# nerfstudio-project/nerfstudio

Hardware: AMD Instinct MI355X
Metric: training rays/sec (4096 rays x 48 samples per GPU) (higher is better)
Workload: dtype f32

## Files before the change

### nerfstudio_amd/csrc/density_mlp.hip

```cpp
#include "common.h"
#include "launch.h"
#include "mfma_chain.h"
#include "proposal_chain.h"

namespace nsamd {

constexpr int kMlpBlock = 256;
constexpr int kMaxBlocks = 768;
constexpr int kDensityActMax = 2048;

__host__ __device__ constexpr int density_partial_stride(int in_dim, int hidden) {
  return (hidden * in_dim + 2 * hidden + 1 + 3) & ~3;
}

template <int IN, int H>
__global__ __launch_bounds__(kMlpBlock) void density_mlp_fwd_kernel(const float* __restrict__ enc,
                                                                    const float* __restrict__ selector, int64_t M,
                                                                    nsamd_density_mlp mlp,
                                                                    float* __restrict__ density,
                                                                    float* __restrict__ pre_out) {
  const float* __restrict__ W0 = mlp.W0;
  const float* __restrict__ b0 = mlp.b0;
  const float* __restrict__ W1 = mlp.W1;
  for (int64_t p = (int64_t)blockIdx.x * kMlpBlock + threadIdx.x; p < M; p += (int64_t)gridDim.x * kMlpBlock) {
    float x[IN];
#pragma unroll
    for (int k = 0; k < IN; ++k) x[k] = enc[(int64_t)k * M + p];
    float out = mlp.b1[0];
    constexpr int JU = (H <= 16) ? H : 4;
#pragma unroll JU
    for (int j = 0; j < H; ++j) {
      float a = b0[j];
#pragma unroll
      for (int k = 0; k < IN; ++k) a = fmaf(W0[j * IN + k], x[k], a);
      out = fmaf(W1[j], fmaxf(a, 0.0f), out);
    }
    const float sel = selector ? selector[p] : 1.0f;
    if (pre_out) pre_out[p] = out;
    density[p] = mlp.average_init_density * expf(out) * sel;
  }
}

template <int LEVELS, int H>
__device__ __forceinline__ void density_point(float x, float y, float z, int64_t p, int64_t M, int transform, const nsamd_aabb& box,
                                              const float2* __restrict__ table, const nsamd_grid& grid,
                                              const nsamd_density_mlp& mlp, float* __restrict__ enc_out,
                                              float* __restrict__ selector_out, float* __restrict__ density,
                                              float* __restrict__ pre_out) {
  constexpr int IN = 2 * LEVELS;
  const float sel = normalise_position(transform, box, x, y, z);
  const uint32_t mask = (1u << grid.log2_table_size) - 1u;
  float2 v[LEVELS][8];
  float w[LEVELS][3];
#pragma unroll
  for (int l = 0; l < LEVELS; ++l) {
    const Cell c = locate_cell(x, y, z, grid.scalings[l]);
    w[l][0] = c.w[0]; w[l][1] = c.w[1]; w[l][2] = c.w[2];
    const float2* __restrict__ tl = table + ((size_t)l << grid.log2_table_size);
#pragma unroll
    for (int k = 0; k < 8; ++k) v[l][k] = tl[corner_index(c, k, mask)];
  }
  float feat[IN];
#pragma unroll
  for (int l = 0; l < LEVELS; ++l) {
#pragma unroll
    for (int f = 0; f < 2; ++f)
      feat[2 * l + f] = trilinear_blend([&](int k) { return f == 0 ? v[l][k].x : v[l][k].y; }, w[l][0], w[l][1], w[l][2]);
  }
  if (enc_out != nullptr) {
#pragma unroll
    for (int k = 0; k < IN; ++k) enc_out[(int64_t)k * M + p] = feat[k];
  }
  if (selector_out != nullptr) selector_out[p] = sel;
  const float* __restrict__ W0 = mlp.W0;
  const float* __restrict__ b0 = mlp.b0;
  const float* __restrict__ W1 = mlp.W1;
  float out = mlp.b1[0];
#pragma unroll
  for (int j = 0; j < H; ++j) {
    float a = b0[j];
#pragma unroll
    for (int k = 0; k < IN; ++k) a = fmaf(W0[j * IN + k], feat[k], a);
    out = fmaf(W1[j], fmaxf(a, 0.0f), out);
  }
  if (pre_out != nullptr) pre_out[p] = out;
  density[p] = mlp.average_init_density * expf(out) * sel;
}

template <int LEVELS, int H>
__global__ __launch_bounds__(kMlpBlock) void density_field_fwd_kernel(nsamd_points P, int64_t M, int transform,
                                                                      nsamd_aabb box, const float2* __restrict__ table,
                                                                      nsamd_grid grid, nsamd_density_mlp mlp,
                                                                      float* __restrict__ enc_out,
                                                                      float* __restrict__ selector_out,
                                                                      float* __restrict__ density,
                                                                      float* __restrict__ pre_out) {
  const int64_t p = (int64_t)blockIdx.x * kMlpBlock + threadIdx.x;
  if (p >= M) return;
  float x, y, z;
  load_position(P, p, x, y, z);
  density_point<LEVELS, H>(x, y, z, p, M, transform, box, table, grid, mlp, enc_out, selector_out, density, pre_out);
}

template <int IN, int H>
__device__ __forceinline__ void density_mlp_bwd_body(
    const float* __restrict__ enc, const float* __restrict__ selector, const float* __restrict__ pre,
    const float* __restrict__ ddensity, int64_t M, const nsamd_density_mlp& mlp, float* __restrict__ denc,
    float* __restrict__ dW0, float* __restrict__ db0, float* __restrict__ dW1, float* __restrict__ db1,
    float* __restrict__ partials, const uint32_t* __restrict__ gate, const uint8_t* __restrict__ ray_mask, int spr,
    int nblocks) {
  if (gate != nullptr && __hip_atomic_load(gate, __ATOMIC_RELAXED, __HIP_MEMORY_SCOPE_AGENT) == 0u) return;
  constexpr int LD = kMlpBlock + 1;
  extern __shared__ __attribute__((aligned(16))) float lds[];
  float* gh_T = lds;
  float* x_T = lds + H * LD;
  float* hg_T = x_T + IN * LD;
  float* gp = hg_T + H * LD;
  constexpr int INP = (IN + 3) & ~3;
  float* w0s = lds + (((2 * H + IN + 1) * LD + 3) & ~3);
  float* b0s = w0s + H * INP;
  float* w1s = b0s + H;
  const int64_t chunks = (M + kMlpBlock - 1) / kMlpBlock;
  const int64_t per_wg = (chunks + nblocks - 1) / nblocks;
  const int64_t c_lo = (int64_t)blockIdx.x * per_wg;
  const int64_t c_hi = c_lo + per_wg < chunks ? c_lo + per_wg : chunks;
  constexpr int kActMax = kDensityActMax;
  uint8_t* act = reinterpret_cast<uint8_t*>(w0s + H * INP + 2 * H);
  const bool use_act = ray_mask != nullptr && per_wg <= kActMax;
  if (use_act) {
    for (int64_t k = threadIdx.x; k < per_wg; k += kMlpBlock) act[k] = 0;
    __syncthreads();
    bool any = false;
    if (c_lo < c_hi) {
      const int64_t p_first = c_lo * kMlpBlock, p_last = (c_hi * kMlpBlock < M ? c_hi * kMlpBlock : M) - 1;
      const int64_t r_first = p_first / spr, r_last = p_last / spr;
      for (int64_t r = r_first + threadIdx.x; r <= r_last; r += kMlpBlock) {
        if (ray_mask[r] != 0) {
          any = true;
          const int64_t q0 = r * spr > p_first ? r * spr : p_first, q1 = (r + 1) * spr - 1 < p_last ? (r + 1) * spr - 1 : p_last;
          for (int64_t c = q0 / kMlpBlock; c <= q1 / kMlpBlock; ++c) act[c - c_lo] = 1;
        }
      }
    }
    if (!__syncthreads_or(any)) {
      if (partials != nullptr) {
        float* row = partials + (size_t)blockIdx.x * density_partial_stride(IN, H);
        for (int e = threadIdx.x; e < H * IN + 2 * H + 1; e += kMlpBlock) row[e] = 0.0f;
      }
      return;
    }
  }
  for (int e = threadIdx.x; e < H * INP; e += kMlpBlock) {
    const int j = e / INP, k = e - j * INP;
    w0s[e] = k < IN ? mlp.W0[j * IN + k] : 0.0f;
  }
  bool w_finite = true;
  for (int e = threadIdx.x; e < H * INP; e += kMlpBlock) w_finite = w_finite && fabsf(w0s[e]) <= 3.4028234663852886e38f;
  for (int e = threadIdx.x; e < H; e += kMlpBlock) {
    b0s[e] = mlp.b0[e];
    w1s[e] = mlp.W1[e];
    w_finite = w_finite && fabsf(b0s[e]) <= 3.4028234663852886e38f && fabsf(w1s[e]) <= 3.4028234663852886e38f;
  }
  const bool may_skip = __syncthreads_and(w_finite) != 0;

  constexpr int NT = H / 16;
  static_assert(H % 16 == 0 && IN <= 16, "dW0 tiling");
  v4f accM[NT];
#pragma unroll
  for (int n = 0; n < NT; ++n) accM[n] = v4f{0.f, 0.f, 0.f, 0.f};
  const int lane = threadIdx.x & 63, wv = threadIdx.x >> 6, jj = lane & 15, gg = lane >> 4;
  float accV = 0.0f;

  float x_next[IN];
  float gd_next = 0.0f, sel_next = 1.0f, pre_next = 0.0f;
  bool act_next = true;
  auto chunk_active = [&](int64_t c) {
    if (ray_mask == nullptr) return true;
    if (use_act) return act[c - c_lo] != 0;
    const int64_t p0 = c * kMlpBlock, p1 = (p0 + kMlpBlock < M ? p0 + kMlpBlock : M) - 1;
    bool any = false;
    for (int64_t r = p0 / spr; r <= p1 / spr; ++r) any = any || ray_mask[r] != 0;
    return any;
  };
  auto fetch = [&](int64_t c) {
    const int64_t p = c * kMlpBlock + threadIdx.x;
    act_next = c < c_hi && chunk_active(c);
    const bool live = act_next && p < M;
#pragma unroll
    for (int k = 0; k < IN; ++k) x_next[k] = live ? enc[(int64_t)k * M + p] : 0.0f;
    gd_next = live ? ddensity[p] : 0.0f;
    sel_next = (live && selector) ? selector[p] : 1.0f;
    pre_next = live ? pre[p] : 0.0f;
  };
  fetch(c_lo);
  for (int64_t c = c_lo; c < c_hi; ++c) {
    if (!act_next) {
      fetch(c + 1);
      continue;
    }
    const int64_t p = c * kMlpBlock + threadIdx.x;
    const bool live = p < M;
    float x[IN];
#pragma unroll
    for (int k = 0; k < IN; ++k) x[k] = x_next[k];
    const float g_pre =
        live ? gd_next * sel_next * mlp.average_init_density * expf(fminf(fmaxf(pre_next, -15.0f), 15.0f)) : 0.0f;
    {
      bool carries = g_pre != 0.0f || !may_skip;
#pragma unroll
      for (int k = 0; k < IN; ++k) carries = carries || !(fabsf(x[k]) <= 3.4028234663852886e38f);
      if (!__syncthreads_or(carries)) {
        if (live) {
#pragma unroll
          for (int k = 0; k < IN; ++k) denc[(int64_t)k * M + p] = 0.0f;
        }
        fetch(c + 1);
        continue;
      }
    }
    float dx[IN];
#pragma unroll
    for (int k = 0; k < IN; ++k) dx[k] = 0.0f;
#pragma unroll 4
    for (int j = 0; j < H; ++j) {
      float wj[INP];
#pragma unroll
      for (int k4 = 0; k4 < INP; k4 += 4) {
        const float4 w4 = *reinterpret_cast<const float4*>(w0s + j * INP + k4);
        wj[k4] = w4.x; wj[k4 + 1] = w4.y; wj[k4 + 2] = w4.z; wj[k4 + 3] = w4.w;
      }
      float a = b0s[j];
#pragma unroll
      for (int k = 0; k < IN; ++k) a = fmaf(wj[k], x[k], a);
      const float gh = (a > 0.0f) ? g_pre * w1s[j] : 0.0f;
      gh_T[j * LD + threadIdx.x] = gh;
      hg_T[j * LD + threadIdx.x] = fmaxf(a, 0.0f) * g_pre;
#pragma unroll
      for (int k = 0; k < IN; ++k) dx[k] = fmaf(gh, wj[k], dx[k]);
    }
#pragma unroll
    for (int k = 0; k < IN; ++k) {
      x_T[k * LD + threadIdx.x] = x[k];
      if (live) denc[(int64_t)k * M + p] = dx[k];
    }
    gp[threadIdx.x] = g_pre;
    __syncthreads();
    fetch(c + 1);
#pragma unroll 4
    for (int q = 0; q < 16; ++q) {
      const int pt = 64 * wv + 4 * q + gg;
      const float b = jj < IN ? x_T[jj * LD + pt] : 0.0f;
#pragma unroll
      for (int n = 0; n < NT; ++n)
        accM[n] = mfma16(gh_T[(16 * n + jj) * LD + pt], b, accM[n]);
    }
    if (threadIdx.x < 2 * H + 1) {
      const float* a = (threadIdx.x < H)       ? gh_T + threadIdx.x * LD
                       : (threadIdx.x < 2 * H) ? hg_T + (threadIdx.x - H) * LD
                                               : gp;
      float s = 0.0f;
#pragma unroll 8
      for (int q = 0; q < kMlpBlock; ++q) s += a[q];
      accV += s;
    }
    __syncthreads();
  }
  float* red = lds;
  for (int e = threadIdx.x; e < H * 16; e += kMlpBlock) red[e] = 0.0f;
  __syncthreads();
  for (int turn = 0; turn < kMlpBlock / 64; ++turn) {
    if (wv == turn) {
#pragma unroll
      for (int n = 0; n < NT; ++n)
#pragma unroll
        for (int r = 0; r < 4; ++r) red[(16 * n + 4 * gg + r) * 16 + jj] += accM[n][r];
    }
    __syncthreads();
  }
  if (partials != nullptr) {
    float* row = partials + (size_t)blockIdx.x * density_partial_stride(IN, H);
    for (int e = threadIdx.x; e < H * IN; e += kMlpBlock) row[e] = red[(e / IN) * 16 + (e % IN)];
    if (threadIdx.x < 2 * H + 1) row[H * IN + threadIdx.x] = accV;
    return;
  }
  for (int e = threadIdx.x; e < H * IN; e += kMlpBlock) unsafeAtomicAdd(dW0 + e, red[(e / IN) * 16 + (e % IN)]);
  if (threadIdx.x < H) unsafeAtomicAdd(db0 + threadIdx.x, accV);
  else if (threadIdx.x < 2 * H) unsafeAtomicAdd(dW1 + (threadIdx.x - H), accV);
  else if (threadIdx.x == 2 * H) unsafeAtomicAdd(db1, accV);
}

template <int IN, int H>
__global__ __launch_bounds__(kMlpBlock) void density_mlp_bwd_kernel(
    const float* __restrict__ enc, const float* __restrict__ selector, const float* __restrict__ pre,
    const float* __restrict__ ddensity, int64_t M, nsamd_density_mlp mlp, float* __restrict__ denc,
    float* __restrict__ dW0, float* __restrict__ db0, float* __restrict__ dW1, float* __restrict__ db1,
    float* __restrict__ partials, const uint32_t* __restrict__ gate, const uint8_t* __restrict__ ray_mask, int spr) {
  density_mlp_bwd_body<IN, H>(enc, selector, pre, ddensity, M, mlp, denc, dW0, db0, dW1, db1, partials, gate, ray_mask, spr,
                              (int)gridDim.x);
}

struct DensityBwdArgs {
  const float* enc;
  const float* selector;
  const float* pre;
  const float* ddensity;
  int64_t M;
  nsamd_density_mlp mlp;
  float* denc;
  float* dW0;
  float* db0;
  float* dW1;
  float* db1;
  float* partials;
  const uint32_t* gate;
  const uint8_t* ray_mask;
  int spr;
  int nblocks;
};

template <int IN, int H>
__global__ __launch_bounds__(kMlpBlock) void density_mlp_bwd_pair_kernel(DensityBwdArgs a, DensityBwdArgs b) {
  if (blockIdx.y == 0) {
    if ((int)blockIdx.x >= a.nblocks) return;
    density_mlp_bwd_body<IN, H>(a.enc, a.selector, a.pre, a.ddensity, a.M, a.mlp, a.denc, a.dW0, a.db0, a.dW1, a.db1,
                                a.partials, a.gate, a.ray_mask, a.spr, a.nblocks);
  } else {
    if ((int)blockIdx.x >= b.nblocks) return;
    density_mlp_bwd_body<IN, H>(b.enc, b.selector, b.pre, b.ddensity, b.M, b.mlp, b.denc, b.dW0, b.db0, b.dW1, b.db1,
                                b.partials, b.gate, b.ray_mask, b.spr, b.nblocks);
  }
}

constexpr int kDwGroups = 16;
__device__ __forceinline__ void density_dw_reduce_body(const float* __restrict__ partials, int rows, int stride, int n_w0,
                                                       int hidden, float* __restrict__ dW0, float* __restrict__ db0,
                                                       float* __restrict__ dW1, float* __restrict__ db1,
                                                       const uint32_t* __restrict__ gate) {
  if (gate != nullptr && __hip_atomic_load(gate, __ATOMIC_RELAXED, __HIP_MEMORY_SCOPE_AGENT) == 0u) return;
  __shared__ float part[kDwGroups][64];
  const int el = threadIdx.x & 63, grp = threadIdx.x >> 6;
  const int e = blockIdx.x * 64 + el;
  const int total = n_w0 + 2 * hidden + 1;
  float s = 0.f;
  if (e < total) {
    for (int b0i = grp; b0i < rows; b0i += kDwGroups * 16) {
      float v[16];
#pragma unroll
      for (int u = 0; u < 16; ++u) {
        const int b = b0i + u * kDwGroups;
        v[u] = partials[(size_t)(b < rows ? b : rows - 1) * stride + e];
      }
#pragma unroll
      for (int u = 0; u < 16; ++u) s += (b0i + u * kDwGroups < rows) ? v[u] : 0.0f;
    }
  }
  part[grp][el] = s;
  __syncthreads();
  if (grp == 0 && e < total) {
    float t = 0.f;
#pragma unroll
    for (int g2 = 0; g2 < kDwGroups; ++g2) t += part[g2][el];
    float* dst = e < n_w0 ? dW0 + e : (e < n_w0 + hidden ? db0 + (e - n_w0) : (e < n_w0 + 2 * hidden ? dW1 + (e - n_w0 - hidden) : db1));
    *dst += t;
  }
}

__global__ __launch_bounds__(64 * kDwGroups) void density_dw_reduce_kernel(const float* __restrict__ partials, int rows,
                                                                            int stride, int n_w0, int hidden,
                                                                            float* __restrict__ dW0,
                                                                            float* __restrict__ db0,
                                                                            float* __restrict__ dW1,
                                                                            float* __restrict__ db1,
                                                                            const uint32_t* __restrict__ gate) {
  density_dw_reduce_body(partials, rows, stride, n_w0, hidden, dW0, db0, dW1, db1, gate);
}

__global__ __launch_bounds__(64 * kDwGroups) void density_dw_reduce_pair_kernel(DensityBwdArgs a, DensityBwdArgs b, int stride,
                                                                                 int n_w0, int hidden) {
  if (blockIdx.y == 0) density_dw_reduce_body(a.partials, a.nblocks, stride, n_w0, hidden, a.dW0, a.db0, a.dW1, a.db1, a.gate);
  else density_dw_reduce_body(b.partials, b.nblocks, stride, n_w0, hidden, b.dW0, b.db0, b.dW1, b.db1, b.gate);
}

template <int IN, int H>
static int launch_fwd(const float* enc, const float* selector, int64_t M, nsamd_density_mlp mlp, float* density,
                      float* pre, hipStream_t stream) {
  const unsigned blocks = (unsigned)min((int64_t)8192, (M + kMlpBlock - 1) / kMlpBlock);
  density_mlp_fwd_kernel<IN, H><<<blocks, kMlpBlock, 0, stream>>>(enc, selector, M, mlp, density, pre);
  NSAMD_CHECK_LAUNCH();
  return NSAMD_OK;
}

#define NSAMD_DENSITY_DISPATCH(CALL)                                  \
  if (mlp.in_dim == 10 && mlp.hidden == 16) return CALL(10, 16);      \
  if (mlp.in_dim == 16 && mlp.hidden == 16) return CALL(16, 16);      \
  if (mlp.in_dim == 10 && mlp.hidden == 64) return CALL(10, 64);      \
  if (mlp.in_dim == 16 && mlp.hidden == 64) return CALL(16, 64);      \
  return NSAMD_ERR_UNSUPPORTED;

template <int IN, int H>
static int launch_bwd(const DensityBwdCall* c, int n, hipStream_t stream) {
  constexpr int stride = density_partial_stride(IN, H);
  constexpr int total = H * IN + 2 * H + 1;
  const size_t lds = sizeof(float) * ((size_t)(2 * H + IN + 1) * (kMlpBlock + 1) + 8 + (size_t)H * (((IN + 3) & ~3) + 2)) +
                     kDensityActMax;
  DensityBwdArgs k[2];
  for (int i = 0; i < n; ++i) {
    const int blocks = (int)min((int64_t)kMaxBlocks, (c[i].M + kMlpBlock - 1) / kMlpBlock);
    float* partials = (c[i].workspace != nullptr && c[i].workspace_floats >= (int64_t)blocks * stride) ? c[i].workspace : nullptr;
    k[i] = DensityBwdArgs{c[i].enc, c[i].selector, c[i].pre, c[i].ddensity, c[i].M, c[i].mlp, c[i].denc, c[i].dW0, c[i].db0,
                          c[i].dW1, c[i].db1, partials, c[i].gate, c[i].ray_mask, c[i].ray_mask ? c[i].spr : 1, blocks};
  }
  const bool pair = n == 2 && k[0].partials != nullptr && k[1].partials != nullptr && k[0].partials != k[1].partials &&
                    k[0].dW0 != k[1].dW0;
  if (n == 2 && !pair) {
    const int rc = launch_bwd<IN, H>(c, 1, stream);
    return rc ? rc : launch_bwd<IN, H>(c + 1, 1, stream);
  }
  if (lds > 64 * 1024) {
    static LdsOptIn opted_in;
    const int rc = lds_opt_in(opted_in, density_mlp_bwd_pair_kernel<IN, H>, lds, density_mlp_bwd_kernel<IN, H>, lds);
    if (rc) return rc;
  }
  const DensityBwdArgs& a = k[0];
  if (pair) {
    density_mlp_bwd_pair_kernel<IN, H><<<dim3((unsigned)max(a.nblocks, k[1].nblocks), 2u), kMlpBlock, lds, stream>>>(a, k[1]);
    NSAMD_CHECK_LAUNCH();
    density_dw_reduce_pair_kernel<<<dim3((total + 63) / 64, 2u), 64 * kDwGroups, 0, stream>>>(a, k[1], stride, H * IN, H);
    NSAMD_CHECK_LAUNCH();
    return NSAMD_OK;
  }
  density_mlp_bwd_kernel<IN, H><<<(unsigned)a.nblocks, kMlpBlock, lds, stream>>>(
      a.enc, a.selector, a.pre, a.ddensity, a.M, a.mlp, a.denc, a.dW0, a.db0, a.dW1, a.db1, a.partials, a.gate, a.ray_mask, a.spr);
  NSAMD_CHECK_LAUNCH();
  if (a.partials != nullptr) {
    density_dw_reduce_kernel<<<(total + 63) / 64, 64 * kDwGroups, 0, stream>>>(a.partials, a.nblocks, stride, H * IN, H, a.dW0,
                                                                             a.db0, a.dW1, a.db1, a.gate);
    NSAMD_CHECK_LAUNCH();
  }
  return NSAMD_OK;
}

static int density_bwd_check(const DensityBwdCall& c) {
  NSAMD_REQUIRE(c.M >= 0);
  NSAMD_REQUIRE(c.ray_mask == nullptr || (c.spr > 0 && c.M % c.spr == 0));
  if (c.M == 0) return NSAMD_OK;
  NSAMD_REQUIRE(c.enc && c.pre && c.ddensity && c.denc && c.dW0 && c.db0 && c.dW1 && c.db1 && c.mlp.W0 && c.mlp.b0 && c.mlp.W1 &&
                c.mlp.b1);
  return NSAMD_OK;
}

int density_bwd_launch(const DensityBwdCall* c, int n, hipStream_t stream) {
  NSAMD_REQUIRE(c != nullptr && (n == 1 || n == 2));
  const nsamd_density_mlp& mlp = c[0].mlp;
  if (n == 2 && (mlp.in_dim != c[1].mlp.in_dim || mlp.hidden != c[1].mlp.hidden || c[0].M <= 0 || c[1].M <= 0 ||
                 density_bwd_check(c[0]) || density_bwd_check(c[1]))) {
    const int rc = density_bwd_launch(c, 1, stream);
    return rc ? rc : density_bwd_launch(c + 1, 1, stream);
  }
  if (n == 1) {
    const int rc = density_bwd_check(c[0]);
    if (rc || c[0].M == 0) return rc;
  }
#define CALL(IN, H) launch_bwd<IN, H>(c, n, stream)
  NSAMD_DENSITY_DISPATCH(CALL)
#undef CALL
}

}

using namespace nsamd;

extern "C" int nsamd_density_mlp_fwd(const float* enc, const float* selector, int64_t M, nsamd_density_mlp mlp,
                                     float* density, float* pre, nsamd_stream_t stream) {
  NSAMD_REQUIRE(M >= 0);
  if (M == 0) return NSAMD_OK;
  NSAMD_REQUIRE(enc && density && mlp.W0 && mlp.b0 && mlp.W1 && mlp.b1);
#define CALL(IN, H) launch_fwd<IN, H>(enc, selector, M, mlp, density, pre, (hipStream_t)stream)
  NSAMD_DENSITY_DISPATCH(CALL)
#undef CALL
}

extern "C" int nsamd_density_field_fwd(nsamd_points pts, int64_t M, int transform, nsamd_aabb aabb, const float* table,
                                       nsamd_grid grid, nsamd_density_mlp mlp, float* enc, float* selector, float* density,
                                       float* pre, nsamd_stream_t stream) {
  NSAMD_REQUIRE(M >= 0);
  if (M == 0) return NSAMD_OK;
  NSAMD_REQUIRE(table && density && mlp.W0 && mlp.b0 && mlp.W1 && mlp.b1);
  NSAMD_REQUIRE(transform >= 0 && transform <= 2);
  if (const int st = check_points(pts, M)) return st;
  if (!table_size_ok(grid)) return NSAMD_ERR_UNSUPPORTED;
  if (mlp.in_dim != 2 * grid.num_levels) return NSAMD_ERR_INVALID_ARG;
  unsigned nb;
  if (grid_blocks((M + kMlpBlock - 1) / kMlpBlock, &nb)) return NSAMD_ERR_UNSUPPORTED;
  const float2* t2 = reinterpret_cast<const float2*>(table);
#define NSAMD_DENSITY_FWD(L_, H_)                                                                                       \
  density_field_fwd_kernel<L_, H_><<<nb, kMlpBlock, 0, (hipStream_t)stream>>>(pts, M, transform, aabb, t2, grid, mlp, \
                                                                                      enc, selector, density, pre)
  if (grid.num_levels == 5 && mlp.hidden == 16) {
    NSAMD_DENSITY_FWD(5, 16);
  } else if (grid.num_levels == 8 && mlp.hidden == 16) {
    NSAMD_DENSITY_FWD(8, 16);
  } else if (grid.num_levels == 5 && mlp.hidden == 64) {
    NSAMD_DENSITY_FWD(5, 64);
  } else if (grid.num_levels == 8 && mlp.hidden == 64) {
    NSAMD_DENSITY_FWD(8, 64);
  } else {
    return NSAMD_ERR_UNSUPPORTED;
  }
#undef NSAMD_DENSITY_FWD
  NSAMD_CHECK_LAUNCH();
  return NSAMD_OK;
}

extern "C" int nsamd_density_mlp_bwd(const float* enc, const float* selector, const float* pre,
                                     const float* ddensity, int64_t M, nsamd_density_mlp mlp, float* denc,
                                     float* dW0, float* db0, float* dW1, float* db1, float* workspace,
                                     int64_t workspace_floats, nsamd_stream_t stream) {
  const DensityBwdCall c{enc, selector, pre, ddensity, M, mlp, denc, dW0, db0, dW1, db1, workspace, workspace_floats,
                         nullptr, nullptr, 1};
  return density_bwd_launch(&c, 1, (hipStream_t)stream);
}

extern "C" int nsamd_density_mlp_bwd_gated(const float* enc, const float* selector, const float* pre,
                                           const float* ddensity, int64_t M, nsamd_density_mlp mlp, float* denc,
                                           float* dW0, float* db0, float* dW1, float* db1, float* workspace,
                                           int64_t workspace_floats, const uint32_t* gate, const uint8_t* ray_mask,
                                           int32_t samples_per_ray, nsamd_stream_t stream) {
  NSAMD_REQUIRE(gate != nullptr);
  const DensityBwdCall c{enc, selector, pre, ddensity, M, mlp, denc, dW0, db0, dW1, db1, workspace, workspace_floats,
                         gate, ray_mask, samples_per_ray};
  return density_bwd_launch(&c, 1, (hipStream_t)stream);
}
```

### nerfstudio_amd/csrc/wave.h

```cpp
#pragma once
#include <hip/hip_runtime.h>

namespace nsamd {

__device__ __forceinline__ int wave_index() { return (int)(threadIdx.x >> 6); }

template <int CTRL, int ROW_MASK>
__device__ __forceinline__ double dpp_move_f64(double v) {
  const unsigned long long b = (unsigned long long)__double_as_longlong(v);
  int lo = (int)(unsigned)(b & 0xffffffffull), hi = (int)(unsigned)(b >> 32);
  lo = __builtin_amdgcn_update_dpp(0, lo, CTRL, ROW_MASK, 0xf, true);
  hi = __builtin_amdgcn_update_dpp(0, hi, CTRL, ROW_MASK, 0xf, true);
  return __longlong_as_double((long long)(((unsigned long long)(unsigned)hi << 32) | (unsigned long long)(unsigned)lo));
}

__device__ __forceinline__ double wave_scan_inclusive_f64(double v) {
  v = v + dpp_move_f64<0x111, 0xf>(v);
  v = v + dpp_move_f64<0x112, 0xf>(v);
  v = v + dpp_move_f64<0x114, 0xf>(v);
  v = v + dpp_move_f64<0x118, 0xf>(v);
  v = v + dpp_move_f64<0x142, 0xa>(v);
  v = v + dpp_move_f64<0x143, 0xc>(v);
  return v;
}

__device__ __forceinline__ double wave_shift_up1_f64(double v) { return dpp_move_f64<0x138, 0xf>(v); }

template <int LANE>
__device__ __forceinline__ double wave_read_f64(double v) {
  const unsigned long long b = (unsigned long long)__double_as_longlong(v);
  const unsigned lo = (unsigned)__builtin_amdgcn_readlane((int)(unsigned)(b & 0xffffffffull), LANE);
  const unsigned hi = (unsigned)__builtin_amdgcn_readlane((int)(unsigned)(b >> 32), LANE);
  return __longlong_as_double((long long)(((unsigned long long)hi << 32) | (unsigned long long)lo));
}

template <int CTRL, int ROW_MASK>
__device__ __forceinline__ uint32_t dpp_move_u32(uint32_t v) {
  return (uint32_t)__builtin_amdgcn_update_dpp(0, (int)v, CTRL, ROW_MASK, 0xf, true);
}
__device__ __forceinline__ uint32_t wave_scan_inclusive_u32(uint32_t v) {
  v += dpp_move_u32<0x111, 0xf>(v);
  v += dpp_move_u32<0x112, 0xf>(v);
  v += dpp_move_u32<0x114, 0xf>(v);
  v += dpp_move_u32<0x118, 0xf>(v);
  v += dpp_move_u32<0x142, 0xa>(v);
  v += dpp_move_u32<0x143, 0xc>(v);
  return v;
}

__device__ __forceinline__ uint32_t row16_max_u32(uint32_t v) {
  v = max(v, dpp_move_u32<0xB1, 0xf>(v));
  v = max(v, dpp_move_u32<0x4E, 0xf>(v));
  v = max(v, dpp_move_u32<0x124, 0xf>(v));
  v = max(v, dpp_move_u32<0x128, 0xf>(v));
  return v;
}

__device__ __forceinline__ uint32_t pair_swap_u32(uint32_t v) {
  return (uint32_t)__builtin_amdgcn_update_dpp(0, (int)v, 0xB1, 0xf, 0xf, false);
}
__device__ __forceinline__ float pair_swap_f32(float v) { return __uint_as_float(pair_swap_u32(__float_as_uint(v))); }

template <int CTRL>
__device__ __forceinline__ float dpp_move_f32(float v) {
  return __uint_as_float((uint32_t)__builtin_amdgcn_update_dpp(0, (int)__float_as_uint(v), CTRL, 0xf, 0xf, false));
}
__device__ __forceinline__ float row16_sum_lane0(float v) {
  v += dpp_move_f32<0xB1>(v);
  v += dpp_move_f32<0x4E>(v);
  v += dpp_move_f32<0x12C>(v);
  v += dpp_move_f32<0x128>(v);
  return v;
}

}
```

Baseline: 6.963 million.

## Spread density-bwd bias reductions across all waves and batch MFMA operand loads

Replaces the per-thread serial 256-element sums for db0/dW1/db1 with a scheme where every wave reduces a strided set of rows cooperatively: four loads per lane, then batched DPP wave scans, with each result owned by one lane. Previously only the first 2H+1 threads did this work while the other waves sat idle. The MFMA loop now loads 8 steps of operands ahead of issuing the MFMAs, giving the scheduler more memory-level parallelism. Launch bounds now request 3 blocks per SIMD, which may raise register pressure or cause spills given the larger operand arrays.

```diff
diff --git a/nerfstudio_amd/csrc/density_mlp.hip b/nerfstudio_amd/csrc/density_mlp.hip
--- a/nerfstudio_amd/csrc/density_mlp.hip
+++ b/nerfstudio_amd/csrc/density_mlp.hip
@@ -2,6 +2,7 @@
 #include "launch.h"
 #include "mfma_chain.h"
 #include "proposal_chain.h"
+#include "wave.h"
 
 namespace nsamd {
 
@@ -116,6 +117,7 @@
   float* x_T = lds + H * LD;
   float* hg_T = x_T + IN * LD;
   float* gp = hg_T + H * LD;
+  constexpr int NV = 2 * H + 1;
   constexpr int INP = (IN + 3) & ~3;
   float* w0s = lds + (((2 * H + IN + 1) * LD + 3) & ~3);
   float* b0s = w0s + H * INP;
@@ -170,6 +172,8 @@
   for (int n = 0; n < NT; ++n) accM[n] = v4f{0.f, 0.f, 0.f, 0.f};
   const int lane = threadIdx.x & 63, wv = threadIdx.x >> 6, jj = lane & 15, gg = lane >> 4;
   float accV = 0.0f;
+  const int own = wv + 4 * lane;
+  const int jb = jj < IN ? jj : 0;
 
   float x_next[IN];
   float gd_next = 0.0f, sel_next = 1.0f, pre_next = 0.0f;
@@ -246,22 +250,44 @@
     gp[threadIdx.x] = g_pre;
     __syncthreads();
     fetch(c + 1);
-#pragma unroll 4
-    for (int q = 0; q < 16; ++q) {
-      const int pt = 64 * wv + 4 * q + gg;
-      const float b = jj < IN ? x_T[jj * LD + pt] : 0.0f;
-#pragma unroll
-      for (int n = 0; n < NT; ++n)
-        accM[n] = mfma16(gh_T[(16 * n + jj) * LD + pt], b, accM[n]);
-    }
-    if (threadIdx.x < 2 * H + 1) {
-      const float* a = (threadIdx.x < H)       ? gh_T + threadIdx.x * LD
-                       : (threadIdx.x < 2 * H) ? hg_T + (threadIdx.x - H) * LD
-                                               : gp;
-      float s = 0.0f;
-#pragma unroll 8
-      for (int q = 0; q < kMlpBlock; ++q) s += a[q];
-      accV += s;
+#pragma unroll
+    for (int q0 = 0; q0 < 16; q0 += 8) {
+      float a[8][NT], b[8];
+#pragma unroll
+      for (int u = 0; u < 8; ++u) {
+        const int pt = 64 * wv + 4 * (q0 + u) + gg;
+        b[u] = x_T[jb * LD + pt];
+#pragma unroll
+        for (int n = 0; n < NT; ++n) a[u][n] = gh_T[(16 * n + jj) * LD + pt];
+      }
+#pragma unroll
+      for (int u = 0; u < 8; ++u) {
+#pragma unroll
+        for (int n = 0; n < NT; ++n) accM[n] = mfma16(a[u][n], b[u], accM[n]);
+      }
+    }
+    {
+      const int wu = __builtin_amdgcn_readfirstlane(wv);
+      constexpr int RPW = (NV + 3) / 4;
+#pragma unroll
+      for (int i0 = 0; i0 < RPW; i0 += 8) {
+        float v[8][4];
+#pragma unroll
+        for (int u = 0; u < 8; ++u) {
+          const int r = min(wu + 4 * (i0 + u), NV - 1);
+          const float* row = r < H ? gh_T + r * LD : hg_T + (r - H) * LD;
+#pragma unroll
+          for (int k = 0; k < 4; ++k) v[u][k] = row[lane + 64 * k];
+        }
+        float t[8];
+#pragma unroll
+        for (int u = 0; u < 8; ++u) t[u] = (v[u][0] + v[u][1]) + (v[u][2] + v[u][3]);
+        wave_sums_f32<8>(t);
+#pragma unroll
+        for (int u = 0; u < 8; ++u) {
+          if (i0 + u < RPW && lane == i0 + u) accV += t[u];
+        }
+      }
     }
     __syncthreads();
   }
@@ -280,17 +306,18 @@
   if (partials != nullptr) {
     float* row = partials + (size_t)blockIdx.x * density_partial_stride(IN, H);
     for (int e = threadIdx.x; e < H * IN; e += kMlpBlock) row[e] = red[(e / IN) * 16 + (e % IN)];
-    if (threadIdx.x < 2 * H + 1) row[H * IN + threadIdx.x] = accV;
+    if (own < NV) row[H * IN + own] = accV;
     return;
   }
   for (int e = threadIdx.x; e < H * IN; e += kMlpBlock) unsafeAtomicAdd(dW0 + e, red[(e / IN) * 16 + (e % IN)]);
-  if (threadIdx.x < H) unsafeAtomicAdd(db0 + threadIdx.x, accV);
-  else if (threadIdx.x < 2 * H) unsafeAtomicAdd(dW1 + (threadIdx.x - H), accV);
-  else if (threadIdx.x == 2 * H) unsafeAtomicAdd(db1, accV);
+  if (own >= NV) return;
+  if (own < H) unsafeAtomicAdd(db0 + own, accV);
+  else if (own < 2 * H) unsafeAtomicAdd(dW1 + (own - H), accV);
+  else unsafeAtomicAdd(db1, accV);
 }
 
 template <int IN, int H>
-__global__ __launch_bounds__(kMlpBlock) void density_mlp_bwd_kernel(
+__global__ __launch_bounds__(kMlpBlock, 3) void density_mlp_bwd_kernel(
     const float* __restrict__ enc, const float* __restrict__ selector, const float* __restrict__ pre,
     const float* __restrict__ ddensity, int64_t M, nsamd_density_mlp mlp, float* __restrict__ denc,
     float* __restrict__ dW0, float* __restrict__ db0, float* __restrict__ dW1, float* __restrict__ db1,
@@ -319,7 +346,7 @@
 };
 
 template <int IN, int H>
-__global__ __launch_bounds__(kMlpBlock) void density_mlp_bwd_pair_kernel(DensityBwdArgs a, DensityBwdArgs b) {
+__global__ __launch_bounds__(kMlpBlock, 3) void density_mlp_bwd_pair_kernel(DensityBwdArgs a, DensityBwdArgs b) {
   if (blockIdx.y == 0) {
     if ((int)blockIdx.x >= a.nblocks) return;
     density_mlp_bwd_body<IN, H>(a.enc, a.selector, a.pre, a.ddensity, a.M, a.mlp, a.denc, a.dW0, a.db0, a.dW1, a.db1,
diff --git a/nerfstudio_amd/csrc/wave.h b/nerfstudio_amd/csrc/wave.h
--- a/nerfstudio_amd/csrc/wave.h
+++ b/nerfstudio_amd/csrc/wave.h
@@ -73,4 +73,26 @@
   return v;
 }
 
+template <int CTRL, int ROW_MASK>
+__device__ __forceinline__ float dpp_move_f32z(float v) {
+  return __uint_as_float(dpp_move_u32<CTRL, ROW_MASK>(__float_as_uint(v)));
 }
+template <int N>
+__device__ __forceinline__ void wave_sums_f32(float* v) {
+#pragma unroll
+  for (int i = 0; i < N; ++i) v[i] += dpp_move_f32z<0x111, 0xf>(v[i]);
+#pragma unroll
+  for (int i = 0; i < N; ++i) v[i] += dpp_move_f32z<0x112, 0xf>(v[i]);
+#pragma unroll
+  for (int i = 0; i < N; ++i) v[i] += dpp_move_f32z<0x114, 0xf>(v[i]);
+#pragma unroll
+  for (int i = 0; i < N; ++i) v[i] += dpp_move_f32z<0x118, 0xf>(v[i]);
+#pragma unroll
+  for (int i = 0; i < N; ++i) v[i] += dpp_move_f32z<0x142, 0xa>(v[i]);
+#pragma unroll
+  for (int i = 0; i < N; ++i) v[i] += dpp_move_f32z<0x143, 0xc>(v[i]);
+#pragma unroll
+  for (int i = 0; i < N; ++i) v[i] = __uint_as_float((uint32_t)__builtin_amdgcn_readlane((int)__float_as_uint(v[i]), 63));
+}
+
+}
```

New measurement: 6.962 million, median of 5. About the same (-0.0%).
